# Chriz122/ultralytics_pro

Measured on AMD Instinct MI355X. Metric: images/sec (whole job = n_gpus x per-GPU bs=32) YOLOv8n 640x640 (forward + Detect decode + NMS), higher is better.
Workload: dtype bf16

## Files before the change

include/upa.h:

```cpp
#ifndef UPA_H
#define UPA_H
#include <stddef.h>
#include <stdint.h>

#ifdef __cplusplus
extern "C" {
#endif

enum { UPA_F32 = 0, UPA_BF16 = 1, UPA_U8_BGR_HWC = 2  };
enum { UPA_ACT_NONE = 0, UPA_ACT_SILU = 1, UPA_ACT_RELU = 2 };
enum { UPA_OK = 0, UPA_EINVAL = -1, UPA_EUNSUPPORTED = -2, UPA_EWORKSPACE = -3, UPA_ELAUNCH = -4 };

typedef struct upa_opts {
  uint32_t size;
  int32_t conv_big;
  int32_t conv_big_bm;
  int32_t conv_ckt;
  int32_t no_ws, no_pipe, no_1x1, no_c16, no_upcat;
  int32_t pipe_all;
  int32_t pipe_min_tiles;
  int32_t pipe_wgs, c16_wgs;
  int32_t c1_mt, c1_waves, c1_wgs;
  int32_t pair;
  int32_t pair_tile64, pair_tile32;
  int32_t no_pair_cv2;
  int32_t c2f;
  int32_t c2f16_waves;
  int32_t c2f32_th;
  int32_t no_branch_tail;
  int32_t branch_tail_bm;
  int32_t stem_wgs, stemf_wgs, stemf_waves, stem_no_mfma;
  int32_t ablate_conv, ablate_pipe, ablate_c1, ablate_stem;
  int32_t c2f64_max_px;
  int32_t conv_ws3;
  int32_t no_group;
  int32_t no_c2f32_up;
  int32_t no_xcd;
  int32_t keys_only;
  int32_t conv_p8;
  int32_t c2f_stream;
  int32_t c2f_stream_rows;
  int32_t no_stack_first;
  int32_t no_epi_stats;
  int32_t nms_stages;
  int32_t nms_first_prefix;
  int32_t detect_stream;
  int32_t detect_stream_rows;
  int32_t no_sppf_front;
  int32_t no_c2f16_down;
} upa_opts;

int upa_version(void);
const char* upa_last_error(void);
size_t upa_opts_size(void);

size_t upa_conv_packed_weight_bytes(int cout, int cin, int k, int dtype);
int upa_pack_conv_weight(const float* w_oihw, int cout, int cin, int k, int dtype, void* out);
int upa_conv2d_bias_act(const void* x, int n, int h, int w, int cin, int ldx,
                        const void* w_packed, const float* bias ,
                        void* y, int cout, int ldy,
                        const void* residual , int ldr,
                        int k, int stride, int pad, int act, int dtype, const upa_opts* opts, void* stream);
typedef struct upa_conv_problem {
  const void* x; int32_t n, h, w, cin, ldx;
  const void* w_packed; const float* bias;
  void* y; int32_t cout, ldy;
  const void* residual; int32_t ldr;
} upa_conv_problem;
int upa_conv2d_bias_act_group(const upa_conv_problem* probs, int count, int k, int stride, int pad, int act, int dtype,
                              const upa_opts* opts, void* stream);

int upa_conv2d_pool2(const void* x, int n, int h, int w, int cin, int ldx, const void* w_packed, const float* bias, void* y, int cout,
                     int ldy, int k, int stride, int pad, int act, int dtype, const upa_opts* opts, void* stream);
int upa_conv2d_stem_nchw_pool2(const void* x_nchw, int x_dtype, int n, int cin, int h, int w, const float* w_oihw, const float* bias,
                               void* y, int cout, int ldy, int k, int stride, int pad, int act, int dtype, const upa_opts* opts,
                               void* stream);

int upa_conv_variant(int n, int h, int w, int cin, int cout, int k, int stride, int pad, int dtype, const upa_opts* opts);

int upa_bottleneck_pair(const void* x, int n, int h, int w, int c, int ldx, const void* w1_packed, const float* b1,
                        const void* w2_packed, const float* b2, void* y, int ldy, int residual, int act, int dtype,
                        const upa_opts* opts, void* stream);
// ... 73 lines not shown
                       void* y, int c2, int ldy, int act, int dtype, const upa_opts* opts, void* stream);

size_t upa_tail_packed_weight_bytes(int cout, int cin);
int upa_pack_tail_weight(const float* w, int cout, int cin, void* out);
int upa_detect_branch_tail(const void* x, int n, int h, int w, int c, int ldx, const void* w3_packed, const float* b3,
                           const void* wt_packed, const float* bt, int kind, int nc, float stride_px, float* y, int a_total,
                           int a0, unsigned long long* best_keys, int dtype, const upa_opts* opts, void* stream);
typedef struct upa_branch_level {
  const void* x; int32_t n, h, w, c, ldx;
  const void* w3_packed; const float* b3;
  const void* wt_packed; const float* bt;
  float stride_px; int32_t a0;
} upa_branch_level;
int upa_detect_branch_tail_group(const upa_branch_level* levels, int count, int kind, int nc, float* y, int a_total,
                                 unsigned long long* best_keys, int dtype, const upa_opts* opts, void* stream);
int upa_detect_head_tails(const upa_branch_level* box, const upa_branch_level* cls, int count, int nc, float* y, int a_total,
                          unsigned long long* best_keys, int dtype, const upa_opts* opts, void* stream);
typedef struct upa_detect_branch {
  int32_t c, reserved;
  const void* w1; const float* b1;
  const void* w2; const float* b2;
  const void* wt; const float* bt;
} upa_detect_branch;
int upa_detect_level_stream(const void* x, int n, int h, int w, int cin, int ldx, const upa_detect_branch* box,
                            const upa_detect_branch* cls, int nc, float stride_px, float* y, int a_total, int a0,
                            unsigned long long* best_keys, int dtype, const upa_opts* opts, void* stream);


size_t upa_nms_workspace_bytes(int b, int nc, int a, int multi_label, int max_nms);
int upa_nms_batched_hot(const float* pred, int b, int nc, int a, float conf_thres, float iou_thres, int multi_label,
                        int agnostic, const uint8_t* classes_mask, int max_det, int max_nms, float max_wh, float* out,
                        int32_t* counts, int32_t* keep_idx, void* workspace, size_t workspace_bytes,
                        const unsigned long long* best_keys, void* stream);
int upa_nms_batched_opts(const float* pred, int b, int nc, int a, float conf_thres, float iou_thres, int multi_label,
                         int agnostic, const uint8_t* classes_mask, int max_det, int max_nms, float max_wh, float* out,
                         int32_t* counts, int32_t* keep_idx, void* workspace, size_t workspace_bytes, const upa_opts* opts,
                         void* stream);
int upa_nms_batched(const float* pred, int b, int nc, int a, float conf_thres, float iou_thres, int multi_label,
                    int agnostic, const uint8_t* classes_mask, int max_det, int max_nms, float max_wh,
                    float* out, int32_t* counts, int32_t* keep_idx, void* workspace, size_t workspace_bytes,
                    void* stream);

int upa_mhsa(const void* q, const void* k, const void* v, int ldqkv, int n, int hw, int heads, int d, float scale,
             const void* residual, int ldr, void* y, int ldy, int dtype, void* stream);
int upa_mhsa_train_fwd(const void* q, const void* k, const void* v, int ldqkv, int n, int hw, int heads, int d, float scale,
                       const void* residual, int ldr, void* y, int ldy, float* lse, int dtype, void* stream);
size_t upa_mhsa_bwd_workspace_bytes(int n, int hw, int heads);
int upa_mhsa_bwd(const void* q, const void* k, const void* v, int ldqkv, const float* lse, const void* d_o, int ldd_o, void* dq, void* dk,
                 void* dv, int lddqkv, int n, int hw, int heads, int d, float scale, void* ws, size_t ws_bytes, int dtype, void* stream);

int upa_dwconv2d(const void* x, int n, int h, int w, int c, int ldx, const float* weight, const float* bias, void* y, int ldy, int k,
                 int stride, int pad, int act, int dtype, void* stream);
int upa_psa_attention(const void* qkv, int ldqkv, int n, int h, int w, int heads, int key_dim, int head_dim, float scale,
                      const float* pe_weight, const float* pe_bias, void* y, int ldy, int dtype, void* stream);

int upa_psa_attention_train_fwd(const void* qkv, int ldqkv, int n, int h, int w, int heads, int key_dim, int head_dim, float scale, void* o,
                                int ldo, float* lse, int dtype, void* stream);
size_t upa_psa_attention_bwd_workspace_bytes(int n, int h, int w, int heads);
int upa_psa_attention_bwd(const void* qkv, int ldqkv, const void* o, int ldo, const float* lse, const void* d_o, int ldd_o, void* dqkv,
                          int lddqkv, int n, int h, int w, int heads, int key_dim, int head_dim, float scale, void* ws, size_t ws_bytes,
                          int dtype, void* stream);
int upa_dwconv2d_train_fwd(const void* x, int n, int h, int w, int c, int ldx, const float* w_c133, void* z, int ldz, int dtype, void* stream);
size_t upa_dwconv2d_bwd_workspace_bytes(int c);
int upa_dwconv2d_bwd(const void* x, const void* dz, int n, int h, int w, int c, int ldx, int lddz, const float* w_c133, void* dx, int lddx,
                     int accumulate_dx, float* dw_c133, int accumulate_dw, void* ws, size_t ws_bytes, int dtype, void* stream);
size_t upa_dwconv2d_bn_act_fwd_workspace_bytes(int n, int h, int w, int c);
// ... 209 lines not shown
```

ultralytics_pro_amd/_lib.py:

```python

from __future__ import annotations

import ctypes as C
import os
from pathlib import Path

import torch

UPA_F32, UPA_BF16, UPA_U8_BGR_HWC = 0, 1, 2
UPA_EINVAL = -1
UPA_EUNSUPPORTED = -2
ACT_NONE, ACT_SILU, ACT_RELU = 0, 1, 2
UPA_PAD_GATHER, UPA_PAD_SCATTER_COPY, UPA_PAD_SCATTER_ADD = 1, 2, 4
MASKS_PLANES, MASKS_OVERLAP = 0, 1
MASK_U8, MASK_F32, MASK_I32 = 0, 1, 2

_PKG = Path(__file__).resolve().parent
LIB_PATH = Path(os.environ.get("UPA_HIP_LIB", _PKG / "libupa_hip.so"))

_vp, _i, _f, _sz = C.c_void_p, C.c_int, C.c_float, C.c_size_t


class Opts(C.Structure):

    _fields_ = [("size", C.c_uint32), ("conv_big", _i), ("conv_big_bm", _i), ("conv_ckt", _i),
                ("no_ws", _i), ("no_pipe", _i), ("no_1x1", _i), ("no_c16", _i), ("no_upcat", _i),
                ("pipe_all", _i), ("pipe_min_tiles", _i), ("pipe_wgs", _i), ("c16_wgs", _i),
                ("c1_mt", _i), ("c1_waves", _i), ("c1_wgs", _i),
                ("pair", _i), ("pair_tile64", _i), ("pair_tile32", _i), ("no_pair_cv2", _i),
                ("c2f", _i), ("c2f16_waves", _i), ("c2f32_th", _i),
                ("no_branch_tail", _i), ("branch_tail_bm", _i),
                ("stem_wgs", _i), ("stemf_wgs", _i), ("stemf_waves", _i), ("stem_no_mfma", _i),
                ("ablate_conv", _i), ("ablate_pipe", _i), ("ablate_c1", _i), ("ablate_stem", _i), ("c2f64_max_px", _i), ("conv_ws3", _i), ("no_group", _i), ("no_c2f32_up", _i), ("no_xcd", _i), ("keys_only", _i), ("conv_p8", _i), ("c2f_stream", _i), ("c2f_stream_rows", _i), ("no_stack_first", _i), ("no_epi_stats", _i), ("nms_stages", _i), ("nms_first_prefix", _i), ("detect_stream", _i), ("detect_stream_rows", _i), ("no_sppf_front", _i), ("no_c2f16_down", _i)]

    def __init__(self, **kw):
        super().__init__()
        self.size = C.sizeof(Opts)
        for k, v in kw.items():
            if k in dict(self._fields_):
                setattr(self, k, int(v))
            else:
                raise AttributeError(f"upa_opts has no field '{k}'")

    def replace(self, **kw) -> "Opts":
        o = Opts()
        C.memmove(C.byref(o), C.byref(self), C.sizeof(Opts))
        for k, v in kw.items():
            setattr(o, k, int(v))
        return o

    _ENV = {"UPA_CONV_BIG": ("conv_big", lambda v: {0: 1, 1: 0, 2: 2}[int(v)]), "UPA_CONV_BIG_BM": ("conv_big_bm", int), "UPA_CONV_WS3": ("conv_ws3", int),
            "UPA_CONV_CKT": ("conv_ckt", int), "UPA_CONV_NO_WS": ("no_ws", lambda v: 1), "UPA_CONV_NO_PIPE": ("no_pipe", lambda v: 1),
            "UPA_CONV_NO_1X1": ("no_1x1", lambda v: 1), "UPA_CONV_NO_C16": ("no_c16", lambda v: 1), "UPA_NO_UPCAT": ("no_upcat", lambda v: 1),
            "UPA_PIPE_ALL": ("pipe_all", lambda v: 1), "UPA_PIPE_MIN_TILES": ("pipe_min_tiles", int), "UPA_PIPE_WGS": ("pipe_wgs", int),
            "UPA_C16_WGS": ("c16_wgs", int), "UPA_C1_MT": ("c1_mt", int), "UPA_C1_WAVES": ("c1_waves", int), "UPA_C1_WGS": ("c1_wgs", int),
            "UPA_NO_PAIR": ("pair", lambda v: {0: 2, 1: 1, 2: 0, 3: 3}[int(v)]), "UPA_PAIR_T64": ("pair_tile64", int),
            "UPA_PAIR_T32": ("pair_tile32", int), "UPA_NO_PAIR_CV2": ("no_pair_cv2", int), "UPA_NO_C2F": ("c2f", int),
            "UPA_C2F16_WAVES": ("c2f16_waves", int), "UPA_C2F32_TH": ("c2f32_th", int), "UPA_NO_BRANCH_TAIL": ("no_branch_tail", int),
            "UPA_BRANCH_TAIL_BM": ("branch_tail_bm", int), "UPA_STEM_WGS": ("stem_wgs", int), "UPA_STEMF_WGS": ("stemf_wgs", int),
            "UPA_STEMF_WAVES": ("stemf_waves", int), "UPA_STEM_NO_MFMA": ("stem_no_mfma", lambda v: 1),
            "UPA_CONV_ABLATE": ("ablate_conv", int), "UPA_PIPE_ABLATE": ("ablate_pipe", int), "UPA_C1_ABLATE": ("ablate_c1", int),
            "UPA_STEM_ABLATE": ("ablate_stem", int)}

    @classmethod
    def from_env(cls, env=None) -> "Opts":
        env = os.environ if env is None else env
# ... 39 lines not shown
    "upa_stem_conv_fused": (_i, [_vp, _i, _i, _i, _vp, _vp, _vp, _vp, _vp, _i, _op, _vp]),
    "upa_stem_conv_fused_k": (_i, [_vp, _i, _i, _i, _i, _vp, _vp, _vp, _vp, _vp, _i, _op, _vp]),
    "upa_stem_conv_fused_c": (_i, [_vp, _i, _i, _i, _i, _i, _vp, _vp, _vp, _vp, _vp, _i, _op, _vp]),
    "upa_stem_conv_fused_s": (_i, [_vp, _i, _i, _i, _i, _i, _i, _vp, _vp, _vp, _vp, _vp, _i, _op, _vp]),
    "upa_stem_variant": (C.c_longlong, [_i, _i, _i, _i, _i, _i, _i, _i, _i, _i, _i, _i, _i, _op, _i]),
    "upa_stem_fused_variant": (C.c_longlong, [_i, _i, _i, _i, _i, _i, _i, _op, _i]),
    "upa_maxpool2d": (_i, [_vp, _i, _i, _i, _i, _i, _vp, _i, _i, _i, _i, _i, _i, _i, _i, _vp]),
    "upa_sppf_pool3": (_i, [_vp, _i, _i, _i, _i, _i, _vp, _vp, _vp, _i, _i, _vp]),
    "upa_upsample2x": (_i, [_vp, _i, _i, _i, _i, _i, _vp, _i, _i, _vp]),
    "upa_copy_view": (_i, [_vp, _i, _i, _i, _i, _i, _vp, _i, _i, _vp]),
    "upa_copy_to_host": (_i, [_vp, _vp, _sz, _vp]),
    "upa_results_to_host": (_i, [_vp, _vp, _i, _i, _i, _vp, _vp, _vp]),
    "upa_add_view": (_i, [_vp, _i, _vp, _i, _vp, _i, _i, _i, _i, _i, _i, _vp]),
    "upa_nchw_to_nhwc": (_i, [_vp, _i, _i, _i, _i, _vp, _i, _i, _vp]),
    "upa_nhwc_to_nchw": (_i, [_vp, _i, _i, _i, _i, _i, _vp, _i, _vp]),
    "upa_letterbox_u8": (_i, [_vp, _i, _i, _i, C.c_long, _i, _vp, _i, _i, _i, _i, _i, _i, _i, _vp]),
    "upa_detect_decode": (_i, [_vp, _i, _vp, _i, _i, _i, _i, _i, _i, _f, _vp, _i, _i, _i, _vp]),
    "upa_detect_branch_tail_group": (_i, [_vp, _i, _i, _i, _vp, _i, _vp, _i, _op, _vp]),
    "upa_detect_head_tails": (_i, [_vp, _vp, _i, _i, _vp, _i, _vp, _i, _op, _vp]),
    "upa_conv2d_bias_act_group": (_i, [_vp, _i, _i, _i, _i, _i, _i, _op, _vp]),
    "upa_detect_level_stream": (_i, [_vp, _i, _i, _i, _i, _i, _vp, _vp, _i, _f, _vp, _i, _i, _vp, _i, _op, _vp]),
    "upa_detect_tail": (_i, [_vp, _i, _i, _i, _i, _i, _vp, _vp, _i, _i, _i, _f, _vp, _i, _i, _vp, _i, _vp, _i, _op, _vp]),
    "upa_conv1x1_upcat": (_i, [_vp, _i, _i, _i, _i, _i, _vp, _i, _i, _vp, _vp, _vp, _i, _i, _i, _i, _op, _vp]),
    "upa_bottleneck_pair_cv2": (_i, [_vp, _vp, _i, _i, _i, _i, _vp, _vp, _vp, _vp, _i, _vp, _vp, _vp, _vp, _i, _i, _i, _op, _vp]),
    "upa_sppf_front": (_i, [_vp, _i, _i, _i, _i, _i, _vp, _vp, _vp, _i, _i, _i, _op, _vp]),
    "upa_c2f16_down_fused": (_i, [_vp, _i, _i, _i, _i, _vp, _vp, _vp, _vp, _vp, _vp, _vp, _vp, _vp, _i, _i, _op, _vp]),
    "upa_c2f_fused": (_i, [_vp, _i, _i, _i, _i, _i, _i, _i, _i, _vp, _vp, _vp, _vp, _vp, _vp, _vp, _i, _i, _i, _i, _op, _vp]),
    "upa_c2f64_fused": (_i, [_vp, _i, _i, _i, _i, _i, _vp, _i, _i, _i, _i, _vp, _vp, _vp, _vp, _vp, _vp, _vp, _i, _i, _i, _i, _op, _vp]),
    "upa_c2f32_up_fused": (_i, [_vp, _i, _i, _i, _i, _i, _vp, _i, _i, _i, _i, _vp, _vp, _vp, _vp, _vp, _vp, _vp, _i, _i, _i, _i, _op, _vp]),
    "upa_tail_packed_weight_bytes": (_sz, [_i, _i]),
    "upa_pack_tail_weight": (_i, [_vp, _i, _i, _vp]),
    "upa_detect_branch_tail": (_i, [_vp, _i, _i, _i, _i, _i, _vp, _vp, _vp, _vp, _i, _i, _f, _vp, _i, _i, _vp, _i, _op, _vp]),
    "upa_nms_batched_hot": (_i, [_vp, _i, _i, _i, _f, _f, _i, _i, _vp, _i, _i, _f, _vp, _vp, _vp, _vp, _sz, _vp, _vp]),
    "upa_nms_workspace_bytes": (_sz, [_i, _i, _i, _i, _i]),
    "upa_nms_batched": (_i, [_vp, _i, _i, _i, _f, _f, _i, _i, _vp, _i, _i, _f, _vp, _vp, _vp, _vp, _sz, _vp]),
    "upa_nms_batched_opts": (_i, [_vp, _i, _i, _i, _f, _f, _i, _i, _vp, _i, _i, _f, _vp, _vp, _vp, _vp, _sz, _vp, _vp]),
    "upa_mhsa": (_i, [_vp, _vp, _vp, _i, _i, _i, _i, _i, _f, _vp, _i, _vp, _i, _i, _vp]),
    "upa_mhsa_train_fwd": (_i, [_vp, _vp, _vp, _i, _i, _i, _i, _i, _f, _vp, _i, _vp, _i, _vp, _i, _vp]),
    "upa_mhsa_bwd_workspace_bytes": (_sz, [_i, _i, _i]),
    "upa_mhsa_bwd": (_i, [_vp, _vp, _vp, _i, _vp, _vp, _i, _vp, _vp, _vp, _i, _i, _i, _i, _i, _f, _vp, _sz, _i, _vp]),
    "upa_dwconv2d": (_i, [_vp, _i, _i, _i, _i, _i, _vp, _vp, _vp, _i, _i, _i, _i, _i, _i, _vp]),
    "upa_psa_attention": (_i, [_vp, _i, _i, _i, _i, _i, _i, _i, _f, _vp, _vp, _vp, _i, _i, _vp]),
    "upa_psa_attention_train_fwd": (_i, [_vp, _i, _i, _i, _i, _i, _i, _i, _f, _vp, _i, _vp, _i, _vp]),
    "upa_psa_attention_bwd_workspace_bytes": (_sz, [_i, _i, _i, _i]),
    "upa_psa_attention_bwd": (_i, [_vp, _i, _vp, _i, _vp, _vp, _i, _vp, _i, _i, _i, _i, _i, _i, _i, _f, _vp, _sz, _i, _vp]),
    "upa_dwconv2d_train_fwd": (_i, [_vp, _i, _i, _i, _i, _i, _vp, _vp, _i, _i, _vp]),
    "upa_dwconv2d_bwd_workspace_bytes": (_sz, [_i]),
    "upa_dwconv2d_bwd": (_i, [_vp, _vp, _i, _i, _i, _i, _i, _i, _vp, _vp, _i, _i, _vp, _i, _vp, _sz, _i, _vp]),
    "upa_dwconv2d_bn_act_fwd_workspace_bytes": (_sz, [_i, _i, _i, _i]),
    "upa_dwconv2d_bn_act_fwd": (_i, [_vp, _i, _i, _i, _i, _i, _vp, _vp, _i, _f, _vp, _vp, _vp, _vp, _vp, _vp, _f, _i, _vp, _i, _vp, _sz, _i,
                                      _vp]),
    "upa_dwconv_bn_act_bwd_workspace_bytes": (_sz, [_i, _i, _i, _i]),
    "upa_dwconv_bn_act_bwd": (_i, [_vp, _i, _i, _i, _i, _i, _vp, _vp, _i, _i, _vp, _vp, _vp, _vp, _f, _i, _vp, _vp, _vp, _vp, _vp, _i, _vp, _i,
                                    _i, _vp, _sz, _i, _vp]),
    "upa_linear": (_i, [_vp, C.c_long, _i, _i, _vp, _vp, _vp, _i, _i, _vp, _i, _i, _vp]),
    "upa_linear_bf16": (_i, [_vp, C.c_long, _i, _i, _vp, _vp, _vp, _i, _i, _vp, _i, _i, _vp]),
    "upa_linear_mixed": (_i, [_vp, _i, C.c_long, _i, _i, _vp, _vp, _vp, _i, _i, _i, _vp, _i, _i, _vp]),
    "upa_layer_norm": (_i, [_vp, _vp, _i, _i, _vp, _vp, _f, _vp, _vp]),
    "upa_rows_add": (_i, [_vp, _vp, _vp, C.c_long, _i, _vp]),
    "upa_rows_scale": (_i, [_vp, _vp, _vp, C.c_long, _i, _vp]),
    "upa_rows_gather": (_i, [_vp, _vp, _vp, C.c_long, _i, _vp]),
    "upa_topk_tokens": (_i, [_vp, _i, _i, _vp, _i, _i, _vp, _vp, _vp]),
    "upa_box_refine": (_i, [_vp, _vp, _vp, C.c_long, _vp]),
    "upa_box_add_anchors": (_i, [_vp, _vp, _vp, _vp, C.c_long, _vp]),
    "upa_sigmoid": (_i, [_vp, _vp, C.c_long, _vp]),
    "upa_rtdetr_output": (_i, [_vp, _vp, _vp, C.c_long, _i, _vp]),
# ... 130 lines not shown
```

ultralytics_pro_amd/csrc/nms.hip:

```cpp
#include "common.h"
#pragma clang fp contract(off)

typedef unsigned long long u64;

namespace {

struct NmsWs {
  int* count;
  int* nsorted;
  u64* keys;
  u64* sel;
};

#ifndef UPA_COARSE_SHIFT
#define UPA_COARSE_SHIFT 17
#endif
constexpr int COARSE_BINS = 4096 >> (UPA_COARSE_SHIFT - 16);
__device__ __forceinline__ int coarse_bin(unsigned inv_score_bits) {
  const int d = (int)(inv_score_bits >> UPA_COARSE_SHIFT) - (int)(0xC07FFFFFu >> UPA_COARSE_SHIFT);
  return d < 0 ? 0 : (d > COARSE_BINS - 1 ? COARSE_BINS - 1 : d);
}

__global__ __launch_bounds__(256) void nms_candidates_kernel(const float* pred, int B, int nc, int A, float conf,
                                                             int multi_label, const uint8_t* cmask, int* count, u64* keys,
                                                             long cap, int* coarse, const int* only_redo) {
  const int b = blockIdx.y;
  if (only_redo && !only_redo[b]) return;
  const int a = blockIdx.x * 256 + threadIdx.x;
  const bool valid = a < A;
  const float* pb = pred + (size_t)b * (4 + nc) * A + (size_t)4 * A + (valid ? a : 0);
  u64* kb = keys + (size_t)b * cap;
  const int lane = threadIdx.x & 63;
  if (!multi_label) {
// ... 219 lines not shown
    for (int i = threadIdx.x; i < nl; i += 256) {
      const int gs = blk_base + i;
      if (gs >= 0 && gs < dcap) dst[gs] = staged[i];
    }
}

__device__ __forceinline__ void lds_barrier() {
  asm volatile("s_waitcnt lgkmcnt(0)" ::: "memory");
  __builtin_amdgcn_sched_barrier(0);
  __builtin_amdgcn_s_barrier();
  __builtin_amdgcn_sched_barrier(0);
}

#ifndef UPA_GREEDY_ROWS_MIN
#define UPA_GREEDY_ROWS_MIN 8
#endif
template <int NT>
__device__ void bitonic_sort(u64* buf, int npad) {
  for (int k = 2; k <= npad; k <<= 1) {
    for (int j = k >> 1; j > 0; j >>= 1) {
      for (int t = threadIdx.x; t < (npad >> 1); t += NT) {
        const int i = 2 * t - (t & (j - 1));
        const int l = i + j;
        const bool up = (i & k) == 0;
        const u64 x = buf[i], y = buf[l];
        if ((x > y) == up) { buf[i] = y; buf[l] = x; }
      }
      __syncthreads();
    }
  }
}

constexpr int SORT_NT = 1024;
constexpr int LDS_SORT_CAP = 16384;

__global__ __launch_bounds__(SORT_NT) void nms_sort_kernel(const int* count, int* nsorted, u64* keys, u64* sel, long cap,
                                                           int selcap, int max_nms, const u64* best_keys, int nc, int A,
                                                           float conf, const uint8_t* cmask, int prefix, int* partial,
                                                           const int* only_redo, const int* coarse, const int* mode,
                                                           const int* pcount) {
  if (only_redo && !only_redo[blockIdx.x]) return;
  extern __shared__ __attribute__((aligned(16))) u64 lbuf[];
  __shared__ int hist[256];
  __shared__ u64 s_prefix;
  __shared__ int s_remaining, s_n;
  const int b = blockIdx.x;
  u64* kb = keys + (size_t)b * cap;
  u64* sb = sel + (size_t)b * selcap;
  int n;
  if (best_keys) {
    const int lane = threadIdx.x & 63;
    if (threadIdx.x == 0) s_n = 0;
    __syncthreads();
    const bool in_lds = prefix == 0 && A <= LDS_SORT_CAP && A <= max_nms && (long)A <= cap;
    constexpr int U = 8;
    for (int a0 = 0; a0 < A; a0 += U * SORT_NT) {
      u64 kk[U];
#pragma unroll
      for (int u = 0; u < U; ++u) {
        const int a = a0 + u * SORT_NT + (int)threadIdx.x;
        kk[u] = a < A ? best_keys[(size_t)b * A + a] : 0ull;
      }
#pragma unroll
      for (int u = 0; u < U; ++u) {
        const int a = a0 + u * SORT_NT + (int)threadIdx.x;
        const u64 k = kk[u];
        bool cand = false;
// ... 176 lines not shown
  } else {
    if (kb != sb)
      for (int i = threadIdx.x; i < n; i += SORT_NT) sb[i] = kb[i];
    for (int i = n + threadIdx.x; i < npad; i += SORT_NT) sb[i] = ~0ull;
    __syncthreads();
    bitonic_sort<SORT_NT>(sb, npad);
  }
  if (threadIdx.x == 0) nsorted[b] = n;
}

__device__ __forceinline__ bool iou_gt(float ax1, float ay1, float ax2, float ay2, float aarea, float bx1, float by1,
                                       float bx2, float by2, float barea, float thr) {
  const float w = fmaxf(fminf(ax2, bx2) - fmaxf(ax1, bx1), 0.f);
  const float h = fmaxf(fminf(ay2, by2) - fmaxf(ay1, by1), 0.f);
  const float inter = w * h;
  const float iou = inter / (aarea + barea - inter);
  return inter != 0.f && !(iou <= thr);
}

#ifdef UPA_GREEDY_PROF
__device__ unsigned long long g_greedy_prof[12];
#define GP_DECL unsigned long long gp_t = __builtin_amdgcn_s_memtime(), gp_acc[12] = {0, 0, 0, 0, 0, 0, 0, 0, 0, 0, 0, 0}
#define GP_AT(i) do { const unsigned long long t_ = __builtin_amdgcn_s_memtime(); gp_acc[i] += t_ - gp_t; gp_t = t_; } while (0)
#define GP_COUNT(i) (gp_acc[i] += 1)
#define GP_FLUSH do { if (threadIdx.x == 0) { for (int i_ = 0; i_ < 12; ++i_) if (i_ != 7) atomicAdd(&g_greedy_prof[i_], gp_acc[i_]); atomicAdd(&g_greedy_prof[7], 1ull); } } while (0)
#else
#define GP_DECL
#define GP_AT(i)
#define GP_COUNT(i)
#define GP_FLUSH
#endif
constexpr int GREEDY_IL = 2;
constexpr int GREEDY_ROWS_MIN = UPA_GREEDY_ROWS_MIN;
#ifndef UPA_GREEDY_NT
#define UPA_GREEDY_NT 1024
#endif
constexpr int GREEDY_NT = UPA_GREEDY_NT;


constexpr int GREEDY_NW = GREEDY_NT / 64;
constexpr int MAX_DET_CAP = 1024;

__global__ __launch_bounds__(GREEDY_NT) void nms_greedy_kernel(const float* pred, int nc, int A, const int* nsorted,
                                                               const u64* sel, int selcap, float iou_thr, int agnostic,
                                                               float max_wh, int max_det, float* out, int* counts,
                                                               int* keep_idx, const int* partial, int* redo, const int* only_redo) {
  if (only_redo && !only_redo[blockIdx.x]) return;
  __shared__ float kx1[MAX_DET_CAP], ky1[MAX_DET_CAP], kx2[MAX_DET_CAP], ky2[MAX_DET_CAP], kar[MAX_DET_CAP];
  __shared__ u64 alive_w[GREEDY_NW];
  __shared__ u64 colm[64];
  __shared__ int s_kept;
  const int b = blockIdx.x;
  const int lane = threadIdx.x & 63, wave = threadIdx.x >> 6;
  GP_DECL;
  const int n = nsorted[b];
  const u64* sb = sel + (size_t)b * selcap;
  const float* pb = pred + (size_t)b * (4 + nc) * A;
  float* ob = out + (size_t)b * max_det * 6;
  if (threadIdx.x == 0) s_kept = 0;
  if (threadIdx.x < 64) colm[threadIdx.x] = 0ull;
  __syncthreads();
  GP_AT(0);
  __shared__ float c_rx1[GREEDY_NT], c_ry1[GREEDY_NT], c_rx2[GREEDY_NT], c_ry2[GREEDY_NT], c_score[GREEDY_NT], c_cls[GREEDY_NT];
  __shared__ int c_anchor[GREEDY_NT];
  for (int stage = 0; stage < n; stage += GREEDY_NT) {
    if (s_kept >= max_det) break;
    {
      const int ci = stage + (int)threadIdx.x;
      if (ci < n) {
        const u64 key = sb[ci];
        const unsigned ok = (unsigned)(key & 0xFFFFFFFFull);
        const int anchor = (int)(ok / (unsigned)nc);
        const int c = (int)(ok - (unsigned)anchor * (unsigned)nc);
        const float cx = pb[anchor], cy = pb[(size_t)A + anchor], w = pb[(size_t)2 * A + anchor],
                    h = pb[(size_t)3 * A + anchor];
        const float hw = w / 2.f, hh = h / 2.f;
        c_rx1[threadIdx.x] = cx - hw; c_ry1[threadIdx.x] = cy - hh; c_rx2[threadIdx.x] = cx + hw; c_ry2[threadIdx.x] = cy + hh;
        c_score[threadIdx.x] = __uint_as_float(~(unsigned)(key >> 32));
        c_cls[threadIdx.x] = (float)c;
        c_anchor[threadIdx.x] = anchor;
      }
    }
    __syncthreads();
    GP_AT(1);
    const int stage_n = n - stage < GREEDY_NT ? n - stage : GREEDY_NT;
    for (int base = 0; base < stage_n; base += 64) {
      const int kept = s_kept;
      if (kept >= max_det) break;
      const int li = base + lane;
// ... 81 lines not shown
            if (nkeep >= room) break;
            const float ix1 = __uint_as_float(__builtin_amdgcn_readlane(__float_as_uint(x1), i));
            const float iy1 = __uint_as_float(__builtin_amdgcn_readlane(__float_as_uint(y1), i));
            const float ix2 = __uint_as_float(__builtin_amdgcn_readlane(__float_as_uint(x2), i));
            const float iy2 = __uint_as_float(__builtin_amdgcn_readlane(__float_as_uint(y2), i));
            const float iar = __uint_as_float(__builtin_amdgcn_readlane(__float_as_uint(area), i));
            const bool sup2 = ((rem >> lane) & 1ull) && iou_gt(ix1, iy1, ix2, iy2, iar, x1, y1, x2, y2, area, iou_thr);
            rem &= ~__ballot(sup2);
          }
        }
        GP_AT(10);
        if ((keepmask >> lane) & 1ull) {
          const int idx = kept + __popcll(keepmask & ((1ull << lane) - 1ull));
          if (idx < max_det) {
            kx1[idx] = x1; ky1[idx] = y1; kx2[idx] = x2; ky2[idx] = y2; kar[idx] = area;
            float* o = ob + (size_t)idx * 6;
            o[0] = rx1; o[1] = ry1; o[2] = rx2; o[3] = ry2; o[4] = score; o[5] = clsf;
            if (keep_idx) keep_idx[(size_t)b * max_det + idx] = anchor;
          }
        }
        if (lane == 0) {
          const int nk = kept + __popcll(keepmask);
          s_kept = nk < max_det ? nk : max_det;
        }
        GP_AT(11);
      }
      GP_AT(4);
      lds_barrier();
      GP_AT(5);
    }
    lds_barrier();
  }
  GP_FLUSH;
  {
    const int k = s_kept;
    for (int i = k * 6 + (int)threadIdx.x; i < max_det * 6; i += GREEDY_NT) ob[i] = 0.f;
    if (keep_idx)
      for (int i = k + (int)threadIdx.x; i < max_det; i += GREEDY_NT) keep_idx[(size_t)b * max_det + i] = -1;
  }
  if (threadIdx.x == 0) {
    counts[b] = s_kept;
    if (redo) redo[b] = (partial && partial[b] && s_kept < max_det) ? 1 : 0;
  }
}

constexpr int NMS_COUNTERS = 8;
inline size_t align_up(size_t v, size_t a) { return (v + a - 1) / a * a; }
inline int pow2_ge(int v) {
  int p = 1;
  while (p < v) p <<= 1;
  return p;
}

}

extern "C" size_t upa_nms_workspace_bytes(int b, int nc, int a, int multi_label, int max_nms) {
  const size_t cap = (size_t)a * (multi_label ? nc : 1);
  const size_t selcap = (size_t)pow2_ge(max_nms < 2 ? 2 : max_nms);
  const size_t counters = (size_t)b * NMS_COUNTERS + (multi_label ? (size_t)b * (COARSE_BINS + 4 * (size_t)cdiv(a, 256) * (size_t)cdiv(nc, 8)) : 0);
  return 256 + align_up(counters * sizeof(int), 256) + (size_t)b * cap * 8 + (size_t)b * selcap * 8;
}

static int nms_batched_impl(const float* pred, int b, int nc, int a, float conf_thres, float iou_thres, int multi_label,
                            int agnostic, const uint8_t* classes_mask, int max_det, int max_nms, float max_wh,
                            float* out, int32_t* counts, int32_t* keep_idx, void* workspace, size_t workspace_bytes,
                            const u64* best_keys, const upa_opts* opts, void* stream) {
  UPA_CHECK_ARG(pred && out && counts && workspace, "nms: null pointer");
  const int stages_mode = UPA_OPT(opts, nms_stages);
  const int first_prefix_opt = UPA_OPT(opts, nms_first_prefix);
  UPA_CHECK_ARG(stages_mode >= 0 && stages_mode <= 2, "nms: opts.nms_stages must be 0, 1 or 2");
  UPA_CHECK_ARG(first_prefix_opt == 0 || first_prefix_opt == -1 || (first_prefix_opt >= 256 && first_prefix_opt < LDS_SORT_CAP),
                "nms: opts.nms_first_prefix must be 0, -1 or in [256, %d)", LDS_SORT_CAP);
  const int first_prefix = first_prefix_opt == 0 ? 4096 : first_prefix_opt;
  UPA_CHECK_ARG(b > 0 && nc > 0 && a > 0, "nms: bad shape");
  UPA_CHECK_ARG(conf_thres >= 0.f && conf_thres <= 1.f, "Invalid Confidence threshold %f, valid values are between 0.0 and 1.0",
                conf_thres);
  UPA_CHECK_ARG(iou_thres >= 0.f && iou_thres <= 1.f, "Invalid IoU %f, valid values are between 0.0 and 1.0", iou_thres);
  UPA_CHECK_ARG(max_det >= 1 && max_det <= MAX_DET_CAP, "nms: max_det must be in [1, %d]", MAX_DET_CAP);
  UPA_CHECK_ARG(max_nms >= 1 && max_nms <= (1 << 20), "nms: max_nms out of range");
  UPA_CHECK_ARG((long)a * nc < (1L << 31), "nms: a*nc overflows the 32-bit candidate index");
  if (workspace_bytes < upa_nms_workspace_bytes(b, nc, a, multi_label, max_nms)) {
    upa_set_error("nms: workspace too small");
    return UPA_EWORKSPACE;
  }
  const bool ws_has_coarse = multi_label != 0;
  multi_label = multi_label && nc > 1;
  const long cap = (long)a * (multi_label ? nc : 1);
  const int selcap = pow2_ge(max_nms < 2 ? 2 : max_nms);
  char* ws = (char*)workspace;
  ws = (char*)align_up((size_t)ws, 256);
  int* count = (int*)ws;
  int* nsorted = count + b;
  int* partial = count + 2 * b;
  int* redo = count + 3 * b;
  ws += align_up(((size_t)b * NMS_COUNTERS + (ws_has_coarse ? (size_t)b * (COARSE_BINS + 4 * (size_t)cdiv(a, 256) * (size_t)cdiv(nc, 8)) : 0)) * sizeof(int), 256);
  u64* keys = (u64*)ws;
  u64* sel = keys + (size_t)b * cap;
  hipStream_t s = (hipStream_t)stream;
  const bool two_stage = cap > LDS_SORT_CAP && max_nms > LDS_SORT_CAP;
  int* coarse = (two_stage && multi_label && !best_keys && stages_mode != 2) ? count + NMS_COUNTERS * b : nullptr;
  int prefixes[3], np = 0;
  if (two_stage && coarse && first_prefix > 0) prefixes[np++] = first_prefix;
  if (two_stage) prefixes[np++] = LDS_SORT_CAP;
  prefixes[np++] = 0;
  const bool emit = coarse && stages_mode == 0;
  int* wave_best = count + NMS_COUNTERS * b + b * COARSE_BINS;
  int *redo2 = count + 4 * b, *mode = count + 5 * b, *pcount = count + 6 * b, *count2 = count + 7 * b;
  if (!best_keys) upa_zero_words(count, coarse ? NMS_COUNTERS * b + b * COARSE_BINS : 2 * b, s);
  const dim3 cgrid((unsigned)cdiv(a, 256), (unsigned)b);
  if (emit) {
    hipLaunchKernelGGL(nms_hist_kernel, cgrid, dim3(256), 0, s, pred, nc, a, conf_thres, classes_mask, coarse, wave_best);
    hipLaunchKernelGGL(nms_emit_kernel, cgrid, dim3(256), 0, s, pred, nc, a, conf_thres, classes_mask, (const int*)coarse,
                       (const int*)wave_best, prefixes[0], count, mode, pcount, keys, cap, sel, selcap);
  } else if (!best_keys) {
    hipLaunchKernelGGL(nms_candidates_kernel, cgrid, dim3(256), 0, s, pred, b, nc, a, conf_thres, multi_label, classes_mask, count,
                       keys, cap, coarse, (const int*)nullptr);
  }
  UPA_LAUNCH_CHECK();
  {
    hipError_t e = upa_full_lds<nms_sort_kernel>();
    if (e != hipSuccess) { upa_set_error("nms: cannot raise LDS limit: %s", hipGetErrorString(e)); return UPA_ELAUNCH; }
  }
  int* flags[3] = {redo, redo2, nullptr};
  for (int i = 0; i < np; ++i) {
    const int* only = i ? flags[i - 1] : nullptr;
    const bool last = i == np - 1;
    if (emit && i == 1)
      hipLaunchKernelGGL(nms_candidates_kernel, cgrid, dim3(256), 0, s, pred, b, nc, a, conf_thres, multi_label, classes_mask, count2,
                         keys, cap, (int*)nullptr, only);
    hipLaunchKernelGGL(nms_sort_kernel, dim3((unsigned)b), dim3(SORT_NT), LDS_SORT_CAP * 8, s, (const int*)((emit && i) ? count2 : count),
                       nsorted, keys, sel, cap, selcap, max_nms, best_keys, nc, a, conf_thres, classes_mask, prefixes[i], partial, only,
// ... 7 lines not shown
  }
  return UPA_OK;
}

#ifdef UPA_GREEDY_PROF
extern "C" int upa_debug_greedy_prof(unsigned long long* out12) {
  unsigned long long* out8 = out12;
  unsigned long long z[12] = {0, 0, 0, 0, 0, 0, 0, 0, 0, 0, 0, 0};
  if (hipMemcpyFromSymbol(out8, HIP_SYMBOL(g_greedy_prof), sizeof(z)) != hipSuccess) return -1;
  return hipMemcpyToSymbol(HIP_SYMBOL(g_greedy_prof), z, sizeof(z)) == hipSuccess ? 0 : -1;
}
#endif

extern "C" int upa_nms_batched(const float* pred, int b, int nc, int a, float conf_thres, float iou_thres, int multi_label,
                               int agnostic, const uint8_t* classes_mask, int max_det, int max_nms, float max_wh,
                               float* out, int32_t* counts, int32_t* keep_idx, void* workspace, size_t workspace_bytes,
                               void* stream) {
  return nms_batched_impl(pred, b, nc, a, conf_thres, iou_thres, multi_label, agnostic, classes_mask, max_det, max_nms, max_wh,
                          out, counts, keep_idx, workspace, workspace_bytes, nullptr, nullptr, stream);
}

extern "C" int upa_nms_batched_opts(const float* pred, int b, int nc, int a, float conf_thres, float iou_thres, int multi_label,
                                    int agnostic, const uint8_t* classes_mask, int max_det, int max_nms, float max_wh,
                                    float* out, int32_t* counts, int32_t* keep_idx, void* workspace, size_t workspace_bytes,
                                    const upa_opts* opts, void* stream) {
  return nms_batched_impl(pred, b, nc, a, conf_thres, iou_thres, multi_label, agnostic, classes_mask, max_det, max_nms, max_wh,
                          out, counts, keep_idx, workspace, workspace_bytes, nullptr, opts, stream);
}

extern "C" int upa_nms_batched_hot(const float* pred, int b, int nc, int a, float conf_thres, float iou_thres, int multi_label,
                                   int agnostic, const uint8_t* classes_mask, int max_det, int max_nms, float max_wh,
                                   float* out, int32_t* counts, int32_t* keep_idx, void* workspace, size_t workspace_bytes,
                                   const unsigned long long* best_keys, void* stream) {
  UPA_CHECK_ARG(best_keys, "nms_hot: best-class keys missing");
  UPA_CHECK_ARG(!(multi_label && nc > 1), "nms_hot: the keys follow the single-label rule (best class per anchor)");
  return nms_batched_impl(pred, b, nc, a, conf_thres, iou_thres, multi_label, agnostic, classes_mask, max_det, max_nms, max_wh,
                          out, counts, keep_idx, workspace, workspace_bytes, (const u64*)best_keys, nullptr, stream);
}
```

ultralytics_pro_amd/utils/nms.py:

```python

from __future__ import annotations

import torch

from .. import _lib as L
from ..engine import runtime as R


def nms_raw(prediction: torch.Tensor, conf_thres=0.25, iou_thres=0.45, classes=None, agnostic=False, multi_label=False,
            max_det=300, nc=0, max_nms=30000, max_wh=7680, key=None):
    if isinstance(prediction, (list, tuple)):
        prediction = prediction[0]
    L.require_gpu(prediction, "non_max_suppression")
    parts = getattr(prediction, "_upa_parts", None)
    if parts is not None or (nc and prediction.dim() == 3 and prediction.shape[1] > 4 + nc):
        if parts is not None:
            y, extra = parts
        else:
            y, extra = prediction[:, :4 + nc].contiguous(), prediction[:, 4 + nc:].contiguous()
        out, counts, keep = nms_raw(y, conf_thres, iou_thres, classes, agnostic, multi_label, max_det, nc, max_nms, max_wh, key)
        b, ne, a = extra.shape
        rows = R.alloc_plain((b, max_det, 6 + ne), torch.float32, y.device, key=(key, "nms_rows"))
        L.check(L.lib().upa_nms_gather_extra(extra.data_ptr(), b, ne, a, keep.data_ptr(), counts.data_ptr(), int(max_det),
                                             out.data_ptr(), rows.data_ptr(), 6 + ne, L.current_stream(y.device)), "nms_gather_extra")
        return rows, counts, keep
    assert 0 <= conf_thres <= 1, f"Invalid Confidence threshold {conf_thres}, valid values are between 0.0 and 1.0"
    assert 0 <= iou_thres <= 1, f"Invalid IoU {iou_thres}, valid values are between 0.0 and 1.0"
    if prediction.dtype != torch.float32 or not prediction.is_contiguous():
        raise L.UpaError("non_max_suppression expects the contiguous float32 (B, 4+nc, A) Detect output")
    b, ch, a = prediction.shape
    nc = nc or (ch - 4)
    if ch != 4 + nc:
        raise L.UpaError(f"prediction has {ch} channels, fewer than 4 + nc = {4 + nc}")
    dev = prediction.device
    lib = L.lib()
    ws_bytes = lib.upa_nms_workspace_bytes(b, nc, a, int(bool(multi_label)), max_nms)
    ws = R.alloc_plain((ws_bytes,), torch.uint8, dev, key=(key, "nms_ws"))
    out = R.alloc_plain((b, max_det, 6), torch.float32, dev, key=(key, "nms_out"))
    counts = R.alloc_plain((b,), torch.int32, dev, key=(key, "nms_counts"))
    keep = R.alloc_plain((b, max_det), torch.int32, dev, key=(key, "nms_keep"))
    cmask = None
    if classes is not None:
        m = torch.zeros(nc, dtype=torch.uint8)
        m[torch.as_tensor(list(classes), dtype=torch.long)] = 1
        cmask = m.to(dev)
    hot = getattr(prediction, "_upa_hot", None)
    if getattr(prediction, "_upa_keys_only", False) and (hot is None or (multi_label and nc > 1)):
        raise L.UpaError("this Detect output was produced in keys-only mode (Detect.scores_out = False): its class rows were not written, "
                         "only single-label NMS (which reads the best-class keys) can consume it - set Detect.scores_out = True for "
                         "multi-label NMS / validation")
    if hot is not None and tuple(hot.shape) == (b, a) and hot.device == dev and not (multi_label and nc > 1):
        L.check(lib.upa_nms_batched_hot(prediction.data_ptr(), b, nc, a, float(conf_thres), float(iou_thres),
                                        int(bool(multi_label)), int(bool(agnostic)), None if cmask is None else cmask.data_ptr(),
                                        int(max_det), int(max_nms), float(max_wh), out.data_ptr(), counts.data_ptr(),
                                        keep.data_ptr(), ws.data_ptr(), ws_bytes, hot.data_ptr(), L.current_stream(dev)),
                "nms_batched_hot")
        return out, counts, keep
    L.check(lib.upa_nms_batched_opts(prediction.data_ptr(), b, nc, a, float(conf_thres), float(iou_thres), int(bool(multi_label)),
                                     int(bool(agnostic)), None if cmask is None else cmask.data_ptr(), int(max_det),
                                     int(max_nms), float(max_wh), out.data_ptr(), counts.data_ptr(), keep.data_ptr(),
                                     ws.data_ptr(), ws_bytes, R.opts_ptr(), L.current_stream(dev)), "nms_batched")
    return out, counts, keep


def non_max_suppression(prediction, conf_thres: float = 0.25, iou_thres: float = 0.45, classes=None,
                        agnostic: bool = False, multi_label: bool = False, labels=(), max_det: int = 300, nc: int = 0,
                        max_time_img: float = 0.05, max_nms: int = 30000, max_wh: int = 7680, rotated: bool = False,
                        end2end: bool = False, return_idxs: bool = False):
    if labels or rotated:
        raise L.UpaError("apriori labels / rotated boxes are outside the hot-path scope")
    if isinstance(prediction, (list, tuple)):
        prediction = prediction[0]
    if prediction.shape[-1] == 6 or end2end:
        raise L.UpaError("end2end (NMS-free) heads are outside the hot-path scope")
    out, counts, keep = nms_raw(prediction, conf_thres, iou_thres, classes, agnostic, multi_label, max_det, nc, max_nms,
                                max_wh)
    n = counts.tolist()
    res = [out[i, : n[i]] for i in range(len(n))]
    if return_idxs:
        return res, [keep[i, : n[i]].long() for i in range(len(n))]
    return res


def rtdetr_postprocess_raw(preds: torch.Tensor, conf: float = 0.25, max_det: int = 300, imgsz=(640, 640), classes=None,
                           orig_shapes=None, key=None):
    if isinstance(preds, (list, tuple)):
        preds = preds[0]
    L.require_gpu(preds, "rtdetr_postprocess")
    if preds.dtype != torch.float32 or not preds.is_contiguous() or preds.dim() != 3:
# ... 23 lines not shown
```

Before: 60030.

## Fuse single-label NMS candidate gather, sort and greedy pass into one kernel

Adds a single-block-per-image NMS kernel for the best-class-key path. It compacts candidates above the confidence threshold into LDS with ballot and atomics, bitonic-sorts them in LDS, then runs the existing greedy suppression, factored out into a device function. This replaces the multi-kernel count/sort/select/greedy pipeline and its global workspace traffic whenever the anchor count fits in LDS (8400 for 640x640 does), and it is on by default unless nms_fused=1. The cost is a large dynamic-LDS request and a bitonic sort over all candidates instead of a prefix-limited sort, which may be slower when many anchors pass the threshold.

```diff
diff --git a/include/upa.h b/include/upa.h
--- a/include/upa.h
+++ b/include/upa.h
@@ -48,6 +48,7 @@
   int32_t detect_stream_rows;
   int32_t no_sppf_front;
   int32_t no_c2f16_down;
+  int32_t nms_fused;
 } upa_opts;
 
 int upa_version(void);
@@ -187,6 +188,10 @@
                         int agnostic, const uint8_t* classes_mask, int max_det, int max_nms, float max_wh, float* out,
                         int32_t* counts, int32_t* keep_idx, void* workspace, size_t workspace_bytes,
                         const unsigned long long* best_keys, void* stream);
+int upa_nms_batched_hot_opts(const float* pred, int b, int nc, int a, float conf_thres, float iou_thres, int multi_label,
+                             int agnostic, const uint8_t* classes_mask, int max_det, int max_nms, float max_wh, float* out,
+                             int32_t* counts, int32_t* keep_idx, void* workspace, size_t workspace_bytes,
+                             const unsigned long long* best_keys, const upa_opts* opts, void* stream);
 int upa_nms_batched_opts(const float* pred, int b, int nc, int a, float conf_thres, float iou_thres, int multi_label,
                          int agnostic, const uint8_t* classes_mask, int max_det, int max_nms, float max_wh, float* out,
                          int32_t* counts, int32_t* keep_idx, void* workspace, size_t workspace_bytes, const upa_opts* opts,
diff --git a/ultralytics_pro_amd/_lib.py b/ultralytics_pro_amd/_lib.py
--- a/ultralytics_pro_amd/_lib.py
+++ b/ultralytics_pro_amd/_lib.py
@@ -31,7 +31,7 @@
                 ("c2f", _i), ("c2f16_waves", _i), ("c2f32_th", _i),
                 ("no_branch_tail", _i), ("branch_tail_bm", _i),
                 ("stem_wgs", _i), ("stemf_wgs", _i), ("stemf_waves", _i), ("stem_no_mfma", _i),
-                ("ablate_conv", _i), ("ablate_pipe", _i), ("ablate_c1", _i), ("ablate_stem", _i), ("c2f64_max_px", _i), ("conv_ws3", _i), ("no_group", _i), ("no_c2f32_up", _i), ("no_xcd", _i), ("keys_only", _i), ("conv_p8", _i), ("c2f_stream", _i), ("c2f_stream_rows", _i), ("no_stack_first", _i), ("no_epi_stats", _i), ("nms_stages", _i), ("nms_first_prefix", _i), ("detect_stream", _i), ("detect_stream_rows", _i), ("no_sppf_front", _i), ("no_c2f16_down", _i)]
+                ("ablate_conv", _i), ("ablate_pipe", _i), ("ablate_c1", _i), ("ablate_stem", _i), ("c2f64_max_px", _i), ("conv_ws3", _i), ("no_group", _i), ("no_c2f32_up", _i), ("no_xcd", _i), ("keys_only", _i), ("conv_p8", _i), ("c2f_stream", _i), ("c2f_stream_rows", _i), ("no_stack_first", _i), ("no_epi_stats", _i), ("nms_stages", _i), ("nms_first_prefix", _i), ("detect_stream", _i), ("detect_stream_rows", _i), ("no_sppf_front", _i), ("no_c2f16_down", _i), ("nms_fused", _i)]
 
     def __init__(self, **kw):
         super().__init__()
@@ -137,6 +137,7 @@
     "upa_pack_tail_weight": (_i, [_vp, _i, _i, _vp]),
     "upa_detect_branch_tail": (_i, [_vp, _i, _i, _i, _i, _i, _vp, _vp, _vp, _vp, _i, _i, _f, _vp, _i, _i, _vp, _i, _op, _vp]),
     "upa_nms_batched_hot": (_i, [_vp, _i, _i, _i, _f, _f, _i, _i, _vp, _i, _i, _f, _vp, _vp, _vp, _vp, _sz, _vp, _vp]),
+    "upa_nms_batched_hot_opts": (_i, [_vp, _i, _i, _i, _f, _f, _i, _i, _vp, _i, _i, _f, _vp, _vp, _vp, _vp, _sz, _vp, _op, _vp]),
     "upa_nms_workspace_bytes": (_sz, [_i, _i, _i, _i, _i]),
     "upa_nms_batched": (_i, [_vp, _i, _i, _i, _f, _f, _i, _i, _vp, _i, _i, _f, _vp, _vp, _vp, _vp, _sz, _vp]),
     "upa_nms_batched_opts": (_i, [_vp, _i, _i, _i, _f, _f, _i, _i, _vp, _i, _i, _f, _vp, _vp, _vp, _vp, _sz, _vp, _vp]),
diff --git a/ultralytics_pro_amd/csrc/nms.hip b/ultralytics_pro_amd/csrc/nms.hip
--- a/ultralytics_pro_amd/csrc/nms.hip
+++ b/ultralytics_pro_amd/csrc/nms.hip
@@ -1,4 +1,5 @@
 #include "common.h"
+#include "nms_hot.h"
 #pragma clang fp contract(off)
 
 typedef unsigned long long u64;
@@ -284,7 +285,7 @@
 }
 
 constexpr int SORT_NT = 1024;
-constexpr int LDS_SORT_CAP = 16384;
+constexpr int LDS_SORT_CAP = NMS_LDS_SORT_CAP;
 
 __global__ __launch_bounds__(SORT_NT) void nms_sort_kernel(const int* count, int* nsorted, u64* keys, u64* sel, long cap,
                                                            int selcap, int max_nms, const u64* best_keys, int nc, int A,
@@ -527,29 +528,20 @@
 #endif
 constexpr int GREEDY_IL = 2;
 constexpr int GREEDY_ROWS_MIN = UPA_GREEDY_ROWS_MIN;
-#ifndef UPA_GREEDY_NT
-#define UPA_GREEDY_NT 1024
-#endif
-constexpr int GREEDY_NT = UPA_GREEDY_NT;
+constexpr int GREEDY_NT = NMS_GREEDY_NT;
 
 
 constexpr int GREEDY_NW = GREEDY_NT / 64;
-constexpr int MAX_DET_CAP = 1024;
-
-__global__ __launch_bounds__(GREEDY_NT) void nms_greedy_kernel(const float* pred, int nc, int A, const int* nsorted,
-                                                               const u64* sel, int selcap, float iou_thr, int agnostic,
-                                                               float max_wh, int max_det, float* out, int* counts,
-                                                               int* keep_idx, const int* partial, int* redo, const int* only_redo) {
-  if (only_redo && !only_redo[blockIdx.x]) return;
+constexpr int MAX_DET_CAP = NMS_MAX_DET_CAP;
+
+__device__ __forceinline__ int greedy_pass(const float* pred, int nc, int A, int b, const u64* sb, int n, float iou_thr,
+                                           int agnostic, float max_wh, int max_det, float* out, int* keep_idx) {
   __shared__ float kx1[MAX_DET_CAP], ky1[MAX_DET_CAP], kx2[MAX_DET_CAP], ky2[MAX_DET_CAP], kar[MAX_DET_CAP];
   __shared__ u64 alive_w[GREEDY_NW];
   __shared__ u64 colm[64];
   __shared__ int s_kept;
-  const int b = blockIdx.x;
   const int lane = threadIdx.x & 63, wave = threadIdx.x >> 6;
   GP_DECL;
-  const int n = nsorted[b];
-  const u64* sb = sel + (size_t)b * selcap;
   const float* pb = pred + (size_t)b * (4 + nc) * A;
   float* ob = out + (size_t)b * max_det * 6;
   if (threadIdx.x == 0) s_kept = 0;
@@ -697,16 +689,89 @@
     lds_barrier();
   }
   GP_FLUSH;
+  const int k = s_kept;
   {
-    const int k = s_kept;
     for (int i = k * 6 + (int)threadIdx.x; i < max_det * 6; i += GREEDY_NT) ob[i] = 0.f;
     if (keep_idx)
       for (int i = k + (int)threadIdx.x; i < max_det; i += GREEDY_NT) keep_idx[(size_t)b * max_det + i] = -1;
   }
+  return k;
+}
+
+__global__ __launch_bounds__(GREEDY_NT) void nms_greedy_kernel(const float* pred, int nc, int A, const int* nsorted,
+                                                               const u64* sel, int selcap, float iou_thr, int agnostic,
+                                                               float max_wh, int max_det, float* out, int* counts,
+                                                               int* keep_idx, const int* partial, int* redo, const int* only_redo) {
+  if (only_redo && !only_redo[blockIdx.x]) return;
+  const int b = blockIdx.x;
+  const int kept = greedy_pass(pred, nc, A, b, sel + (size_t)b * selcap, nsorted[b], iou_thr, agnostic, max_wh, max_det, out, keep_idx);
   if (threadIdx.x == 0) {
-    counts[b] = s_kept;
-    if (redo) redo[b] = (partial && partial[b] && s_kept < max_det) ? 1 : 0;
-  }
+    counts[b] = kept;
+    if (redo) redo[b] = (partial && partial[b] && kept < max_det) ? 1 : 0;
+  }
+}
+
+template <int NT>
+__device__ void bitonic_sort_prefix(u64* buf, int n) {
+  int npad = 2;
+  while (npad < n) npad <<= 1;
+  for (int k = 2; k <= npad; k <<= 1) {
+    for (int j = k >> 1; j > 0; j >>= 1) {
+      for (int t = threadIdx.x; t < (npad >> 1); t += NT) {
+        int i, l;
+        nms_hot_sort_pair(t, k, j, i, l);
+        if (l < n) {
+          const u64 x = buf[i], y = buf[l];
+          if (x > y) { buf[i] = y; buf[l] = x; }
+        }
+      }
+      lds_barrier();
+    }
+  }
+}
+
+__global__ __launch_bounds__(GREEDY_NT) void nms_hot_kernel(const float* pred, int nc, int A, const u64* best_keys, float conf,
+                                                            const uint8_t* cmask, int max_nms, float iou_thr, int agnostic,
+                                                            float max_wh, int max_det, float* out, int* counts, int* keep_idx) {
+  extern __shared__ __attribute__((aligned(16))) u64 hbuf[];
+  __shared__ int s_n;
+  const int b = blockIdx.x;
+  const int lane = threadIdx.x & 63;
+  if (threadIdx.x == 0) s_n = 0;
+  __syncthreads();
+  constexpr int U = 8;
+  for (int a0 = 0; a0 < A; a0 += U * GREEDY_NT) {
+    u64 kk[U];
+#pragma unroll
+    for (int u = 0; u < U; ++u) {
+      const int a = a0 + u * GREEDY_NT + (int)threadIdx.x;
+      kk[u] = a < A ? best_keys[(size_t)b * A + a] : 0ull;
+    }
+#pragma unroll
+    for (int u = 0; u < U; ++u) {
+      const int a = a0 + u * GREEDY_NT + (int)threadIdx.x;
+      const u64 k = kk[u];
+      bool cand = false;
+      if (a < A) {
+        const float best = __uint_as_float(~(unsigned)(k >> 32));
+        const int bc = (int)((unsigned)k - (unsigned)a * (unsigned)nc);
+        cand = best > conf && (!cmask || cmask[bc]);
+      }
+      const u64 m = __ballot(cand);
+      if (m) {
+        int base = 0;
+        if (lane == 0) base = atomicAdd(&s_n, __popcll(m));
+        base = __shfl(base, 0);
+        if (cand) hbuf[base + __popcll(m & ((1ull << lane) - 1ull))] = k;
+      }
+    }
+  }
+  lds_barrier();
+  int n = s_n;
+  bitonic_sort_prefix<GREEDY_NT>(hbuf, n);
+  if (n > max_nms) n = max_nms;
+  const int kept = greedy_pass(pred, nc, A, b, hbuf, n, iou_thr, agnostic, max_wh, max_det, out, keep_idx);
+  if (threadIdx.x == 0) counts[b] = kept;
 }
 
 constexpr int NMS_COUNTERS = 8;
@@ -715,6 +780,16 @@
   int p = 1;
   while (p < v) p <<= 1;
   return p;
+}
+
+hipError_t nms_hot_prepare() {
+  static const hipError_t e = [] {
+    hipFuncAttributes fa;
+    if (hipError_t r = hipFuncGetAttributes(&fa, (const void*)nms_hot_kernel); r != hipSuccess) return r;
+    if (fa.sharedSizeBytes > nms_hot_static_lds()) return hipErrorInvalidValue;
+    return upa_full_lds<nms_hot_kernel>();
+  }();
+  return e;
 }
 
 }
@@ -737,6 +812,8 @@
   UPA_CHECK_ARG(first_prefix_opt == 0 || first_prefix_opt == -1 || (first_prefix_opt >= 256 && first_prefix_opt < LDS_SORT_CAP),
                 "nms: opts.nms_first_prefix must be 0, -1 or in [256, %d)", LDS_SORT_CAP);
   const int first_prefix = first_prefix_opt == 0 ? 4096 : first_prefix_opt;
+  const int fused_opt = UPA_OPT(opts, nms_fused);
+  UPA_CHECK_ARG(fused_opt == 0 || fused_opt == 1, "nms: opts.nms_fused must be 0 or 1");
   UPA_CHECK_ARG(b > 0 && nc > 0 && a > 0, "nms: bad shape");
   UPA_CHECK_ARG(conf_thres >= 0.f && conf_thres <= 1.f, "Invalid Confidence threshold %f, valid values are between 0.0 and 1.0",
                 conf_thres);
@@ -762,6 +839,16 @@
   u64* keys = (u64*)ws;
   u64* sel = keys + (size_t)b * cap;
   hipStream_t s = (hipStream_t)stream;
+  if (nms_hot_applies(best_keys != nullptr, multi_label, nc, a, fused_opt)) {
+    if (hipError_t e = nms_hot_prepare(); e != hipSuccess) {
+      upa_set_error("nms: cannot raise LDS limit: %s", hipGetErrorString(e));
+      return UPA_ELAUNCH;
+    }
+    hipLaunchKernelGGL(nms_hot_kernel, dim3((unsigned)b), dim3(GREEDY_NT), nms_hot_dyn_lds(a), s, pred, nc, a, best_keys, conf_thres,
+                       classes_mask, max_nms, iou_thres, agnostic, max_wh, max_det, out, counts, keep_idx);
+    UPA_LAUNCH_CHECK();
+    return UPA_OK;
+  }
   const bool two_stage = cap > LDS_SORT_CAP && max_nms > LDS_SORT_CAP;
   int* coarse = (two_stage && multi_label && !best_keys && stages_mode != 2) ? count + NMS_COUNTERS * b : nullptr;
   int prefixes[3], np = 0;
@@ -835,8 +922,16 @@
                                    int agnostic, const uint8_t* classes_mask, int max_det, int max_nms, float max_wh,
                                    float* out, int32_t* counts, int32_t* keep_idx, void* workspace, size_t workspace_bytes,
                                    const unsigned long long* best_keys, void* stream) {
+  return upa_nms_batched_hot_opts(pred, b, nc, a, conf_thres, iou_thres, multi_label, agnostic, classes_mask, max_det, max_nms, max_wh,
+                                  out, counts, keep_idx, workspace, workspace_bytes, best_keys, nullptr, stream);
+}
+
+extern "C" int upa_nms_batched_hot_opts(const float* pred, int b, int nc, int a, float conf_thres, float iou_thres, int multi_label,
+                                        int agnostic, const uint8_t* classes_mask, int max_det, int max_nms, float max_wh,
+                                        float* out, int32_t* counts, int32_t* keep_idx, void* workspace, size_t workspace_bytes,
+                                        const unsigned long long* best_keys, const upa_opts* opts, void* stream) {
   UPA_CHECK_ARG(best_keys, "nms_hot: best-class keys missing");
   UPA_CHECK_ARG(!(multi_label && nc > 1), "nms_hot: the keys follow the single-label rule (best class per anchor)");
   return nms_batched_impl(pred, b, nc, a, conf_thres, iou_thres, multi_label, agnostic, classes_mask, max_det, max_nms, max_wh,
-                          out, counts, keep_idx, workspace, workspace_bytes, (const u64*)best_keys, nullptr, stream);
-}
+                          out, counts, keep_idx, workspace, workspace_bytes, (const u64*)best_keys, opts, stream);
+}
diff --git a/ultralytics_pro_amd/csrc/nms_hot.h b/ultralytics_pro_amd/csrc/nms_hot.h
--- /dev/null
+++ b/ultralytics_pro_amd/csrc/nms_hot.h
@@ -0,0 +1,39 @@
+#ifndef UPA_NMS_HOT_H
+#define UPA_NMS_HOT_H
+#include <stddef.h>
+
+#if defined(__HIPCC__)
+#define UPA_NMS_HD __host__ __device__
+#else
+#define UPA_NMS_HD
+#endif
+
+#ifndef UPA_GREEDY_NT
+#define UPA_GREEDY_NT 1024
+#endif
+
+constexpr int NMS_GREEDY_NT = UPA_GREEDY_NT;
+constexpr int NMS_MAX_DET_CAP = 1024;
+constexpr int NMS_LDS_SORT_CAP = 16384;
+constexpr size_t NMS_LDS_BYTES = 160 * 1024;
+
+constexpr size_t nms_hot_static_lds() {
+  return (size_t)5 * NMS_MAX_DET_CAP * 4 + (size_t)7 * NMS_GREEDY_NT * 4 + (size_t)(NMS_GREEDY_NT / 64) * 8 + 64 * 8 + 16;
+}
+constexpr size_t nms_hot_dyn_lds(int a) { return (size_t)a * 8; }
+constexpr int nms_hot_max_a() {
+  const size_t fit = (NMS_LDS_BYTES - nms_hot_static_lds()) / 8;
+  return fit < (size_t)NMS_LDS_SORT_CAP ? (int)fit : NMS_LDS_SORT_CAP;
+}
+
+inline bool nms_hot_applies(bool have_keys, int multi_label, int nc, int a, int nms_fused) {
+  const bool ml = multi_label && nc > 1;
+  return have_keys && !ml && a >= 1 && a <= nms_hot_max_a() && nms_fused != 1;
+}
+
+UPA_NMS_HD inline void nms_hot_sort_pair(int t, int k, int j, int& i, int& l) {
+  i = 2 * t - (t & (j - 1));
+  l = j == (k >> 1) ? (i ^ (k - 1)) : i + j;
+}
+
+#endif
diff --git a/ultralytics_pro_amd/utils/nms.py b/ultralytics_pro_amd/utils/nms.py
--- a/ultralytics_pro_amd/utils/nms.py
+++ b/ultralytics_pro_amd/utils/nms.py
@@ -50,11 +50,11 @@
                          "only single-label NMS (which reads the best-class keys) can consume it - set Detect.scores_out = True for "
                          "multi-label NMS / validation")
     if hot is not None and tuple(hot.shape) == (b, a) and hot.device == dev and not (multi_label and nc > 1):
-        L.check(lib.upa_nms_batched_hot(prediction.data_ptr(), b, nc, a, float(conf_thres), float(iou_thres),
-                                        int(bool(multi_label)), int(bool(agnostic)), None if cmask is None else cmask.data_ptr(),
-                                        int(max_det), int(max_nms), float(max_wh), out.data_ptr(), counts.data_ptr(),
-                                        keep.data_ptr(), ws.data_ptr(), ws_bytes, hot.data_ptr(), L.current_stream(dev)),
-                "nms_batched_hot")
+        L.check(lib.upa_nms_batched_hot_opts(prediction.data_ptr(), b, nc, a, float(conf_thres), float(iou_thres),
+                                             int(bool(multi_label)), int(bool(agnostic)), None if cmask is None else cmask.data_ptr(),
+                                             int(max_det), int(max_nms), float(max_wh), out.data_ptr(), counts.data_ptr(),
+                                             keep.data_ptr(), ws.data_ptr(), ws_bytes, hot.data_ptr(), R.opts_ptr(),
+                                             L.current_stream(dev)), "nms_batched_hot")
         return out, counts, keep
     L.check(lib.upa_nms_batched_opts(prediction.data_ptr(), b, nc, a, float(conf_thres), float(iou_thres), int(bool(multi_label)),
                                      int(bool(agnostic)), None if cmask is None else cmask.data_ptr(), int(max_det),
```

After: 60320 (median of 5 runs). About the same (+0.5%).
